# secondChoice/flink

Measured on AMD Instinct MI355X. Metric: records/sec/node, keyed TUMBLE SUM/COUNT/AVG at 1/2/4/8 GPU; % of HBM peak, higher is better.
Workload: dtype f64

## Files before the change

flink_amd/csrc/fg_kernels.hip:

```cpp
#include <hip/hip_runtime.h>

#include <algorithm>
#include <cstdio>
#include <vector>

#include <type_traits>

#include "fg_kernels.h"

namespace fg {

thread_local LaunchEvents g_launch_ev;

typedef long long RecV2 __attribute__((ext_vector_type(2)));
typedef const RecV2 __attribute__((address_space(1)))* GlobalRec;

__device__ __forceinline__ longlong2 ld2(const void* q) {
    const RecV2 v = *static_cast<const RecV2*>(q);
    return make_longlong2(v.x, v.y);
}
__device__ __forceinline__ void st2(void* q, longlong2 a) {
    RecV2 v;
    v.x = a.x;
    v.y = a.y;
// ... 3396 lines not shown
    int32_t t_base, ng;
    int32_t gk, wave, W;
    uint32_t* q;
    int32_t gsz;
    uint32_t xn[kTileTPL];
    uint32_t g_len[kTileTPL], g_st[kTileTPL], g_tot, b;
};
template <bool MAX>
__device__ __forceinline__ uint32_t dpp_op(uint32_t a, uint32_t b) { return MAX ? (a > b ? a : b) : a + b; }
template <bool MAX>
__device__ __forceinline__ uint32_t wave_incl_scan(uint32_t v) {
    v = dpp_op<MAX>(v, (uint32_t)__builtin_amdgcn_update_dpp(0, (int)v, 0x111, 0xf, 0xf, false));
    v = dpp_op<MAX>(v, (uint32_t)__builtin_amdgcn_update_dpp(0, (int)v, 0x112, 0xf, 0xf, false));
    v = dpp_op<MAX>(v, (uint32_t)__builtin_amdgcn_update_dpp(0, (int)v, 0x114, 0xf, 0xf, false));
    v = dpp_op<MAX>(v, (uint32_t)__builtin_amdgcn_update_dpp(0, (int)v, 0x118, 0xf, 0xf, false));
    v = dpp_op<MAX>(v, (uint32_t)__builtin_amdgcn_update_dpp(0, (int)v, 0x142, 0xa, 0xf, false));
    v = dpp_op<MAX>(v, (uint32_t)__builtin_amdgcn_update_dpp(0, (int)v, 0x143, 0xc, 0xf, false));
    return v;
}
__device__ __forceinline__ uint32_t wave_shr1(uint32_t v) {
    return (uint32_t)__builtin_amdgcn_update_dpp(0, (int)v, 0x138, 0xf, 0xf, false);
}

__device__ __forceinline__ int32_t tile_walk_grab(TileWalk& w, int lane) {
    if (!w.q) return w.wave + w.W * (w.gk++);
    uint32_t g = 0;
    if (lane == 0) g = atomicAdd(w.q, 1u);
    return (int32_t)__builtin_amdgcn_readfirstlane(g);
}
__device__ __forceinline__ void tile_walk_begin(TileWalk& w, const TilePass& tp, int32_t cb, int wave, int W,
                                                int lane, int32_t t_lo, int32_t t_hi, uint32_t* q = nullptr) {
    w.col = tp.dt + (int64_t)cb * tp.nt;
    w.rec = tp.rec;
    w.n = (uint32_t)tp.n;
    w.bad = false;
    w.nt = t_hi;
    const int32_t per = (t_hi - t_lo + W - 1) / W;
    w.gsz = per >= kTileGroup ? kTileGroup : (per + kTileTPL - 1) / kTileTPL * kTileTPL;
    if (w.gsz < kTileTPL) w.gsz = kTileTPL;
    w.t_base = t_lo;
    w.ng = t_hi > t_lo ? (t_hi - t_lo + w.gsz - 1) / w.gsz : 0;
    w.gk = 0;
    w.wave = wave;
    w.W = W;
    w.q = w.ng >= 4 * W ? q : nullptr;
    const int32_t g0 = tile_walk_grab(w, lane);
    w.tn = g0 < w.ng ? t_lo + g0 * w.gsz : t_hi;
#pragma unroll
    for (int q4 = 0; q4 < kTileTPL; q4++) {
        const int t = w.tn + lane * kTileTPL + q4;
        const bool ok = t < w.nt && lane * kTileTPL + q4 < w.gsz;
        const uint32_t x = gbl(w.col)[ok ? t : 0];
        w.xn[q4] = ok ? x : 0u;
        w.g_len[q4] = w.g_st[q4] = 0;
    }
    w.g_tot = w.b = 0;
}
__device__ __forceinline__ bool tile_walk_next(TileWalk& w, uint8_t* fm, uint32_t* dl, int lane,
                                               int32_t (&kr)[kTileRpl], int64_t (&vr)[kTileRpl], uint32_t& nrec) {
    static_assert(kTileRpl == 4, "one fragment-map word per lane");
    bool done = false;
    while (w.b >= w.g_tot) {
        w.t0 = w.tn;
        if (w.t0 >= w.nt) {
            done = true;
            break;
        }
        const int32_t gn = tile_walk_grab(w, lane);
        w.tn = gn < w.ng ? w.t_base + gn * w.gsz : w.nt;
        uint32_t base[kTileTPL], sum = 0;
#pragma unroll
        for (int q = 0; q < kTileTPL; q++) {
            const int t = w.t0 + lane * kTileTPL + q;
            const uint32_t x = w.xn[q];
            const int tn = w.tn + lane * kTileTPL + q;
            const bool okn = tn < w.nt && lane * kTileTPL + q < w.gsz;
            const uint32_t xn = gbl(w.col)[okn ? tn : 0];
            w.xn[q] = okn ? xn : 0u;
            w.g_len[q] = x >> 16;
            base[q] = (uint32_t)t * (uint32_t)kTileRecs + (x & 0xffffu);
            w.g_st[q] = sum;
            sum += w.g_len[q];
        }
        uint32_t inc = wave_incl_scan<false>(sum);
        asm volatile("" : "+v"(inc));
        const uint32_t ex = inc - sum;
        w.g_tot = (uint32_t)__builtin_amdgcn_readlane((int)inc, 63);
        w.b = 0;
        wave_lds_sync();
#pragma unroll
        for (int q = 0; q < kTileTPL; q++) {
            w.g_st[q] += ex;
            dl[lane * kTileTPL + q] = base[q] - w.g_st[q];
        }
    }
    if (done) {
        w.b = w.g_tot = 0;
    }
    uint32_t* fm32 = reinterpret_cast<uint32_t*>(fm);
    fm32[lane] = 0;
    wave_lds_sync();
#pragma unroll
    for (int q = 0; q < kTileTPL; q++) {
        const uint32_t st = w.g_st[q], len = w.g_len[q];
        if (len > 0 && st < w.b + kTileWin && st + len > w.b) fm[st > w.b ? st - w.b : 0] = (uint8_t)(lane * kTileTPL + q);
    }
    wave_lds_sync();
    const uint32_t e4 = fm32[lane];
    uint32_t e0 = e4 & 255u, e1 = (e4 >> 8) & 255u, e2 = (e4 >> 16) & 255u, e3 = e4 >> 24;
    e1 = e1 > e0 ? e1 : e0;
    e2 = e2 > e1 ? e2 : e1;
    e3 = e3 > e2 ? e3 : e2;
    const uint32_t pre = wave_shr1(wave_incl_scan<true>(e3));
    e0 = e0 > pre ? e0 : pre;
    e1 = e1 > pre ? e1 : pre;
    e2 = e2 > pre ? e2 : pre;
    e3 = e3 > pre ? e3 : pre;
    fm32[lane] = e0 | e1 << 8 | e2 << 16 | e3 << 24;
    wave_lds_sync();
    nrec = w.g_tot - w.b < (uint32_t)kTileWin ? w.g_tot - w.b : (uint32_t)kTileWin;
    uint32_t fq[kTileRpl], dq[kTileRpl];
#pragma unroll
    for (int u = 0; u < kTileRpl; u++) fq[u] = fm[lane + 64 * u] & (uint32_t)(kTileGroup - 1);
#pragma unroll
    for (int u = 0; u < kTileRpl; u++) dq[u] = dl[fq[u]];
#pragma unroll
    for (int u = 0; u < kTileRpl; u++) {
        const uint32_t jr = lane + 64 * u;
        uint32_t src = jr < nrec ? dq[u] + w.b + jr : 0u;
        if (src >= w.n) {
#ifdef FG_DEBUG_WALK
            if (!w.bad)
                printf("walk: lane %d u %d jr %u nrec %u b %u g_tot %u t0 %d nt %d n %u src %u fm %u dl %u "
                       "g_st %u %u g_len %u %u xn %u %u\n", lane, u, jr, nrec, w.b, w.g_tot, w.t0, w.nt, w.n, src,
                       (uint32_t)fm[jr], dl[fm[jr]], w.g_st[0], w.g_st[1], w.g_len[0], w.g_len[1], w.xn[0], w.xn[1]);
#endif
            w.bad = true;
            src = 0;
        }
#if defined(FG_DIAG_FIRE) && (FG_DIAG_FIRE & 1)
        kr[u] = (int32_t)((src * 2654435761u) >> 20);
        vr[u] = (int64_t)src;
#else
        const Rec12 r = ld_tile_rec(w.rec, (uint64_t)src);
        kr[u] = (int32_t)r.k;
        vr[u] = rec12_val(r);
#endif
    }
    w.b += kTileWin;
    return !done;
}

__global__ __launch_bounds__(256) void k_selftest_scan(const uint32_t* in, uint32_t* out) {
    const uint32_t v = in[threadIdx.x];
    const uint32_t a = wave_incl_scan<false>(v);
    const uint32_t m = wave_incl_scan<true>(v & 255u);
    out[3 * threadIdx.x] = a;
    out[3 * threadIdx.x + 1] = m;
    out[3 * threadIdx.x + 2] = wave_shr1(m);
}
__global__ __launch_bounds__(64) void k_selftest_walk(TilePass tp, uint32_t cap, uint32_t* out, uint32_t* n_out,
                                                      unsigned int* bad) {
    __shared__ __attribute__((aligned(16))) uint8_t s_fm[kTileWin];
    __shared__ uint32_t s_dl[kTileGroup];
    const int lane = threadIdx.x;
    const int32_t cb = blockIdx.x;
    TileWalk w;
    tile_walk_begin(w, tp, cb, 0, 1, lane, 0, tp.nt);
    int32_t kr[kTileRpl];
    int64_t vr[kTileRpl];
    uint32_t nrec = 0, pos = 0;
    while (tile_walk_next(w, s_fm, s_dl, lane, kr, vr, nrec)) {
#pragma unroll
        for (int u = 0; u < kTileRpl; u++) {
            const uint32_t jr = lane + 64 * u;
            if (jr < nrec && pos + jr < cap) out[(uint64_t)cb * cap + pos + jr] = (uint32_t)kr[u];
        }
        pos += nrec;
    }
    if (lane == 0) n_out[cb] = pos;
    if (__ballot(w.bad) != 0 && lane == 0) atomicOr(bad, 1u);
}
__global__ void k_selftest_fill(uint32_t* rec, uint64_t n) {
    for (uint64_t i = blockIdx.x * (uint64_t)blockDim.x + threadIdx.x; i < n; i += (uint64_t)gridDim.x * blockDim.x) {
        rec[3 * i] = (uint32_t)i;
        rec[3 * i + 1] = 0u;
        rec[3 * i + 2] = (uint32_t)i;
    }
}

int run_selftest(int device, char* msg, size_t cap_msg) {
    auto say = [&](const char* m) {
        if (msg && cap_msg) snprintf(msg, cap_msg, "%s", m);
    };
    if (hipSetDevice(device) != hipSuccess) {
        say("hipSetDevice failed");
        return 1;
    }
    uint64_t x = 0x5EEDF11Cull;
    auto rnd = [&]() {
        x = x * 6364136223846793005ull + 1442695040888963407ull;
        return (uint32_t)(x >> 33);
    };
    std::vector<uint32_t> in(256), got(3 * 256);
    for (auto& v : in) v = rnd() & 1023u;
    constexpr int NT = 300, NB = 3;
    std::vector<uint32_t> dt((size_t)NB * NT);
    std::vector<std::vector<uint32_t>> want(NB);
    for (int t = 0; t < NT; t++) {
        uint32_t off = rnd() % 64;
        for (int b = 0; b < NB; b++) {
            const uint32_t len = rnd() % 5 == 0 ? 0 : rnd() % 21;
            dt[(size_t)b * NT + t] = off | len << 16;
            for (uint32_t i = 0; i < len; i++) want[b].push_back((uint32_t)t * (uint32_t)kTileRecs + off + i);
            off += len;
        }
    }
    const uint64_t nrec = (uint64_t)NT * kTileRecs;
    uint32_t cap = 0;
    for (auto& v : want) cap = std::max<uint32_t>(cap, (uint32_t)v.size());
    void *d_in = nullptr, *d_out = nullptr, *d_rec = nullptr, *d_dt = nullptr, *d_w = nullptr, *d_n = nullptr,
         *d_bad = nullptr;
    int rc = 0;
    const char* what = nullptr;
    auto cleanup = [&]() {
        for (void* q : {d_in, d_out, d_rec, d_dt, d_w, d_n, d_bad})
            if (q) (void)hipFree(q);
    };
    if (hipMalloc(&d_in, 4 * 256) != hipSuccess || hipMalloc(&d_out, 4 * 3 * 256) != hipSuccess ||
        hipMalloc(&d_rec, 12 * nrec) != hipSuccess || hipMalloc(&d_dt, 4 * dt.size()) != hipSuccess ||
        hipMalloc(&d_w, 4 * (size_t)NB * cap + 4) != hipSuccess || hipMalloc(&d_n, 4 * NB) != hipSuccess ||
        hipMalloc(&d_bad, 4) != hipSuccess) {
        cleanup();
        say("self-check: device allocation failed");
        return 1;
    }
    (void)hipMemcpy(d_in, in.data(), 4 * 256, hipMemcpyHostToDevice);
    (void)hipMemcpy(d_dt, dt.data(), 4 * dt.size(), hipMemcpyHostToDevice);
    (void)hipMemset(d_bad, 0, 4);
    k_selftest_scan<<<1, 256>>>(static_cast<const uint32_t*>(d_in), static_cast<uint32_t*>(d_out));
    k_selftest_fill<<<256, 256>>>(static_cast<uint32_t*>(d_rec), nrec);
    TilePass tp{};
    tp.rec = d_rec;
    tp.dt = static_cast<const uint32_t*>(d_dt);
    tp.n = (int64_t)nrec;
    tp.nt = NT;
    tp.mt = NT;
    tp.nc = NB;
    k_selftest_walk<<<NB, 64>>>(tp, cap, static_cast<uint32_t*>(d_w), static_cast<uint32_t*>(d_n),
                                static_cast<unsigned int*>(d_bad));
    std::vector<uint32_t> walk((size_t)NB * cap), wn(NB);
    unsigned int bad = 0;
    if (hipDeviceSynchronize() != hipSuccess || hipMemcpy(got.data(), d_out, 4 * 3 * 256, hipMemcpyDeviceToHost) ||
        hipMemcpy(walk.data(), d_w, 4 * walk.size(), hipMemcpyDeviceToHost) ||
        hipMemcpy(wn.data(), d_n, 4 * NB, hipMemcpyDeviceToHost) || hipMemcpy(&bad, d_bad, 4, hipMemcpyDeviceToHost)) {
        cleanup();
        say("self-check: a kernel or copy failed");
        return 1;
    }
    cleanup();
    for (int wv = 0; wv < 4 && !what; wv++) {
        uint32_t a = 0, m = 0, prev = 0;
        for (int l = 0; l < 64; l++) {
            const uint32_t v = in[64 * wv + l];
            a += v;
            m = (v & 255u) > m ? (v & 255u) : m;
            const uint32_t* o = &got[3 * (64 * wv + l)];
            if (o[0] != a) what = "self-check: the DPP add scan (wave_incl_scan) is wrong";
            else if (o[1] != m) what = "self-check: the DPP max scan (wave_incl_scan) is wrong";
            else if (o[2] != (l ? prev : 0u)) what = "self-check: the DPP lane shift (wave_shr1) is wrong";
            if (what) break;
            prev = m;
        }
    }
    for (int b = 0; b < NB && !what; b++) {
        if (wn[b] != want[b].size()) what = "self-check: the tile walk visited a wrong number of records";
        for (size_t i = 0; !what && i < want[b].size(); i++)
            if (walk[(size_t)b * cap + i] != want[b][i]) what = "self-check: the tile walk read a wrong record";
    }
    if (!what && bad) what = "self-check: the tile walk addressed a record past its pass";
    if (what) {
        say(what);
        rc = 1;
    } else {
        say("ok");
    }
    return rc;
}

template <int VTC, bool TAB, int SM>
__global__ __launch_bounds__(kTileFireThreads) void k_tile_fire(TileFire fa) {
    const TileFire& f = fa;
    constexpr bool HOT = SM == 2;
    constexpr int T = kTileFireThreads, W = T / 64, S = kTileSlots;
    constexpr int kRounds = S / T + 1;
    static_assert(S % T == 0 && (S & (S - 1)) == 0, "table rounds");
    constexpr int kDummy = S + 1;
    __shared__ __attribute__((aligned(16))) int32_t t_key[S + 2];
    __shared__ uint32_t t_cs[S + 2];
    __shared__ unsigned long long t_v[S + 2];
    __shared__ __attribute__((aligned(16))) uint8_t s_fm[W][kTileWin];
    __shared__ uint32_t s_dl[W][kTileGroup];
    __shared__ uint32_t s_grp[kRounds * W];
    __shared__ uint16_t s_map[S + 1];
    __shared__ unsigned int s_flags;
    __shared__ uint32_t s_total;
    __shared__ unsigned long long s_out_base;
    __shared__ uint32_t s_rc[kTileMaxRegions];
    __shared__ uint32_t s_rb[kTileMaxRegions];
    __shared__ uint32_t s_gnext[kMaxTilePasses];
    const MergeParams& p = f.m;
    const bool dst = TAB && p.has_dst != 0;
    const int tid = threadIdx.x, lane = tid & 63, wave = tid >> 6;
#ifdef FG_STAMPS
    unsigned long long fst_acc[8] = {0, 0, 0, 0, 0, 0, 0, 0};
    unsigned long long fst_prev = __builtin_amdgcn_s_memtime();
#define FSTAMP(i)                                                     \
    do {                                                              \
        const unsigned long long now_ = __builtin_amdgcn_s_memtime(); \
        fst_acc[i] += now_ - fst_prev;                                \
        fst_prev = now_;                                              \
    } while (0)
#define FWAIT(kk, vv) asm volatile("" ::"v"(kk[kTileRpl - 1]), "v"(vv[kTileRpl - 1]))
#else
#define FSTAMP(i) \
    do {          \
    } while (0)
#define FWAIT(kk, vv) \
    do {              \
    } while (0)
#endif
    const int vt = VTC >= 0 ? VTC : p.val_type;
    const int64_t vinit = lds_repr(vt, val_identity(vt));
    const int sub = p.region_bits - f.tbits;
    const bool retry = p.retry_list != nullptr;
    const bool split = SM != 0 && f.split != 0;
    const bool merge = split && f.merge != 0;
    __shared__ int s_item;
    const int NI = retry ? p.n_retry
                   : merge ? (int)*gbl(f.sp.n_split)
                   : split ? (int)*gbl(f.sp.n_items)
                           : 1 << (f.tbits - kTileBits);
    const int G = gridDim.x;
    const bool xcd = !retry && !split && G % 8 == 0;
    for (int k = 0;; k++) {
        const int b = (int)blockIdx.x;
        int x = xcd ? k * G + (b % 8) * (G / 8) + b / 8 : b + k * G;
        if (split && !merge) {
            if (tid == 0) s_item = (int)atomicAdd(f.sp.next_item, 1u);
            __syncthreads();
            x = s_item;
            if (x >= NI) break;
        } else if (k * G >= NI) {
            break;
        }
        bool live = x < NI;
#if !defined(FG_FIRE_HOIST)
        const TileFire& f = (&fa)[opaque_zero()];
        const MergeParams& p = f.m;
#endif
        int r_lo = 0, r_hi = 0, item = 0;
        int32_t g_lo = 0, g_hi = 0x7fffffff, part = -1;
        int32_t mc0 = 0, mck = 0;
        if (live) {
            if (merge) {
                item = f.sp.split_b[x];
                mc0 = f.sp.split_c0[x];
                mck = f.sp.split_k[x];
                r_lo = item << (sub + kTileBits);
                r_hi = (item + 1) << (sub + kTileBits);
                live = *gbl(&f.sp.bfail[item]) == 0u;
            } else if (retry) {
                r_lo = gbl(p.retry_list)[x];
                r_hi = r_lo + 1;
                item = r_lo >> (sub + kTileBits);
            } else if (split) {
                const TileItem it = f.sp.items[x];
                item = it.bucket;
                g_lo = it.g_lo;
                g_hi = it.g_hi;
                part = it.part;
                r_lo = item << (sub + kTileBits);
                r_hi = (item + 1) << (sub + kTileBits);
            } else {
                item = x;
                r_lo = x << (sub + kTileBits);
                r_hi = (x + 1) << (sub + kTileBits);
            }
        }
        const bool to_part = split && !merge && part >= 0;
        for (int i = tid; i <= S + 1; i += T) {
            t_key[i] = kEmpty32;
            t_cs[i] = 0;
            t_v[i] = (unsigned long long)vinit;
        }
        if (TAB)
            for (int i = tid; i < kTileMaxRegions; i += T) s_rc[i] = 0;
        if (tid < kMaxTilePasses) s_gnext[tid] = 0;
        if (tid == 0) s_flags = 0;
        __syncthreads();
        FSTAMP(0);
        bool full = false;
#if defined(FG_DIAG_FIRE)
        uint64_t diag_sink = 0;
#endif
        auto slot_of = [&](int32_t key) -> int {
            if (key == kEmpty32) return S;
            uint32_t home = __umulhi((uint32_t)key * 0x9E3779B1u, (uint32_t)(S / 4)) * 4;
            for (int probe = 0; probe < S / 4; probe++) {
                const int4 q4 = *reinterpret_cast<const int4*>(&t_key[home]);
                const int32_t qq[4] = {q4.x, q4.y, q4.z, q4.w};
                int hit = -1, emp = -1;
#pragma unroll
                for (int z = 3; z >= 0; z--) {
                    if (qq[z] == key) hit = z;
                    if (qq[z] == kEmpty32) emp = z;
                }
                if (hit >= 0 && (emp < 0 || hit < emp)) return (int)home + hit;
                if (emp >= 0) {
                    const int old = atomicCAS(&t_key[home + emp], kEmpty32, key);
                    if (old == kEmpty32 || old == key) return (int)home + emp;
                    continue;
                }
                home = (home + 4) & (S - 1);
            }
            return -1;
        };
        if (TAB && p.n_src > 0 && !to_part) {
            constexpr int cap = kRegionCap;
            const int nreg = r_hi - r_lo, nrange = live ? p.n_src * nreg : 0;
            if (wave == 0) {
                constexpr int RPL = kTileMaxRegions / 64;
                uint32_t c[RPL], x = 0;
#pragma unroll
                for (int q = 0; q < RPL; q++) {
                    const int g = RPL * lane + q;
                    c[q] = g < nrange ? gbl(src_at(p, g / nreg).counts)[r_lo + g % nreg] : 0u;
                    x += c[q];
                }
                for (int off = 1; off < 64; off <<= 1) {
                    const uint32_t y = __shfl_up(x, off);
                    if (lane >= off) x += y;
                }
                uint32_t ex = x;
#pragma unroll
                for (int q = 0; q < RPL; q++) ex -= c[q];
#pragma unroll
                for (int q = 0; q < RPL; q++) {
                    if (RPL * lane + q < nrange) s_rb[RPL * lane + q] = ex;
                    ex += c[q];
                }
                if (lane == 63) s_total = x;
            }
            __syncthreads();
            const uint32_t NE = nrange ? s_total : 0u;
            for (uint32_t i0 = 0; !p.src_narrow && i0 < NE; i0 += kSrcU * T) {
                int64_t mk[kSrcU], cs[kSrcU], v[kSrcU];
#pragma unroll
                for (int u = 0; u < kSrcU; u++) {
                    const uint32_t i = i0 + u * T + tid;
                    mk[u] = cs[u] = v[u] = 0;
                    if (i >= NE) continue;
                    int lo = 0, hi = nrange;
                    while (hi - lo > 1) {
                        const int mid = (lo + hi) >> 1;
                        if (s_rb[mid] <= i) lo = mid;
                        else hi = mid;
                    }
                    const auto base = gbl(src_at(p, lo / nreg).base + (int64_t)(r_lo + lo % nreg) * 4 * cap);
                    const uint32_t e = i - s_rb[lo];
                    mk[u] = base[e];
                    cs[u] = base[cap + e];
                    v[u] = base[3 * cap + e];
                }
#pragma unroll
                for (int u = 0; u < kSrcU; u++) {
                    if (i0 + u * T + tid >= NE) continue;
                    const int sl = slot_of((int32_t)key_of(mk[u]));
                    if (sl < 0) {
                        full = true;
                        continue;
                    }
                    atomicAdd(&t_cs[sl], (uint32_t)cs[u]);
                    lds_val(&t_v[sl], v[u], vt, true);
                }
            }
            for (uint32_t i0 = 0; p.src_narrow && i0 < NE; i0 += kSrcU * T) {
                int64_t cs[kSrcU], v[kSrcU];
                int32_t mk[kSrcU];
#pragma unroll
                for (int u = 0; u < kSrcU; u++) {
                    const uint32_t i = i0 + u * T + tid;
                    mk[u] = 0;
                    cs[u] = v[u] = 0;
                    if (i >= NE) continue;
                    int lo = 0, hi = nrange;
                    while (hi - lo > 1) {
                        const int mid = (lo + hi) >> 1;
                        if (s_rb[mid] <= i) lo = mid;
                        else hi = mid;
                    }
                    const TableRef sr = src_at(p, lo / nreg);
                    const auto base = gbl(sr.base + (int64_t)(r_lo + lo % nreg) * 4 * cap);
                    const uint32_t e = i - s_rb[lo];
                    const bool nar = sr.narrow != 0;
                    mk[u] = tab_key32(base, cap, e, nar);
                    cs[u] = tab_cs(base, cap, e, nar);
                    v[u] = tab_v(base, cap, e, nar);
                }
#pragma unroll
                for (int u = 0; u < kSrcU; u++) {
                    if (i0 + u * T + tid >= NE) continue;
                    const int sl = slot_of(mk[u]);
                    if (sl < 0) {
                        full = true;
                        continue;
                    }
                    atomicAdd(&t_cs[sl], (uint32_t)cs[u]);
                    lds_val(&t_v[sl], v[u], vt, true);
                }
            }
        }
        FSTAMP(4);
        if (live && merge) {
            constexpr int kPartU = 4;
            for (int c0 = mc0; c0 < mc0 + mck; c0 += kTileMaxRegions) {
                const int nc = min(kTileMaxRegions, mc0 + mck - c0);
                __syncthreads();
                if (wave == 0) {
                    constexpr int RPL = kTileMaxRegions / 64;
                    uint32_t c[RPL], x = 0;
#pragma unroll
                    for (int q = 0; q < RPL; q++) {
                        const int g = RPL * lane + q;
                        c[q] = 0;
                        if (g < nc) {
                            const uint32_t off = f.sp.part_off[c0 + g], n = f.sp.part_n[c0 + g];
                            if ((uint64_t)off + n <= (uint64_t)f.sp.part_cap) c[q] = n;
                            else atomicOr(p.overflow, 2u);
                        }
                        x += c[q];
                    }
                    for (int off = 1; off < 64; off <<= 1) {
                        const uint32_t y = __shfl_up(x, off);
                        if (lane >= off) x += y;
                    }
                    uint32_t ex = x;
#pragma unroll
                    for (int q = 0; q < RPL; q++) ex -= c[q];
#pragma unroll
                    for (int q = 0; q < RPL; q++) {
                        if (RPL * lane + q < nc) s_rb[RPL * lane + q] = ex;
                        ex += c[q];
                    }
                    if (lane == 63) s_total = x;
                }
                __syncthreads();
                const uint32_t NE = s_total;
                for (uint32_t i0 = 0; i0 < NE; i0 += kPartU * T) {
                    int32_t pk[kPartU];
                    uint32_t pc[kPartU];
                    unsigned long long pv[kPartU];
#pragma unroll
                    for (int u = 0; u < kPartU; u++) {
                        const uint32_t i = i0 + u * T + tid;
                        pk[u] = kEmpty32;
                        pc[u] = 0;
                        pv[u] = 0;
                        if (i >= NE) continue;
                        int lo = 0, hi = nc;
                        while (hi - lo > 1) {
                            const int mid = (lo + hi) >> 1;
                            if (s_rb[mid] <= i) lo = mid;
                            else hi = mid;
                        }
                        const uint32_t e = f.sp.part_off[c0 + lo] + (i - s_rb[lo]);
                        pk[u] = f.sp.p_key[e];
                        pc[u] = f.sp.p_cs[e];
                        pv[u] = f.sp.p_v[e];
                    }
#pragma unroll
                    for (int u = 0; u < kPartU; u++) {
                        if (i0 + u * T + tid >= NE) continue;
                        const int sl = slot_of(pk[u]);
                        if (sl < 0) {
                            full = true;
                            continue;
                        }
                        atomicAdd(&t_cs[sl], pc[u]);
                        lds_val(&t_v[sl], lds_repr(vt, (int64_t)pv[u]), vt, true);
                    }
                }
            }
        } else if (live) {
            auto insert_plain = [&](auto FULL, auto RETRY, const int32_t (&kr)[kTileRpl], const int64_t (&vr)[kTileRpl],
                                    uint32_t nrec) {
#if defined(FG_DIAG_FIRE) && (FG_DIAG_FIRE & 2)
#pragma unroll
                for (int u = 0; u < kTileRpl; u++)
                    if (lane + 64 * u < nrec) diag_sink ^= (uint64_t)kr[u] ^ (uint64_t)vr[u];
                return;
#endif
                uint32_t hm[kTileRpl];
                int4 bq[kTileRpl];
#pragma unroll
                for (int u = 0; u < kTileRpl; u++) {
                    hm[u] = __umulhi((uint32_t)kr[u] * 0x9E3779B1u, (uint32_t)(S / 4)) * 4;
                    bq[u] = *reinterpret_cast<const int4*>(&t_key[hm[u]]);
                }
#pragma unroll
                for (int u = 0; u < kTileRpl; u++) {
                    if (!decltype(FULL)::value && lane + 64 * u >= nrec) continue;
                    const int32_t key = kr[u];
                    if (decltype(RETRY)::value && retry &&
                        (int)((uint64_t)mix_of((int64_t)key) >> (64 - p.region_bits)) != r_lo)
                        continue;
                    int sl = -1;
                    if (key == kEmpty32) {
                        sl = S;
                    } else {
                        uint32_t home = hm[u];
                        int4 q4 = bq[u];
                        for (int probe = 0; probe < S / 4; probe++) {
                            const int32_t qq[4] = {q4.x, q4.y, q4.z, q4.w};
                            int hit = -1, emp = -1;
#pragma unroll
                            for (int z = 3; z >= 0; z--) {
                                if (qq[z] == key) hit = z;
                                if (qq[z] == kEmpty32) emp = z;
                            }
                            if (hit >= 0 && (emp < 0 || hit < emp)) {
                                sl = (int)home + hit;
                                break;
                            }
                            if (emp >= 0) {
                                const int old = atomicCAS(&t_key[home + emp], kEmpty32, key);
                                if (old == kEmpty32 || old == key) {
                                    sl = (int)home + emp;
                                    break;
                                }
                            } else {
                                home = (home + 4) & (S - 1);
                            }
                            q4 = *reinterpret_cast<const int4*>(&t_key[home]);
                        }
                    }
                    if (sl < 0) {
                        full = true;
                        continue;
                    }
                    atomicAdd(&t_cs[sl], 1u);
                    lds_val(&t_v[sl], vr[u], vt, true);
                }
            };
            auto insert_hot = [&](const int32_t (&kr)[kTileRpl], const int64_t (&vr)[kTileRpl], uint32_t nrec) {
                const bool hot = vt >= 0 && vt <= 2;
                uint32_t hm[kTileRpl];
                int4 bq[kTileRpl];
                int sl[kTileRpl];
                uint32_t cn[kTileRpl];
                int64_t va[kTileRpl];
#pragma unroll
                for (int u = 0; u < kTileRpl; u++) {
                    hm[u] = __umulhi((uint32_t)kr[u] * 0x9E3779B1u, (uint32_t)(S / 4)) * 4;
                    bq[u] = *reinterpret_cast<const int4*>(&t_key[hm[u]]);
                    cn[u] = 1u;
                    va[u] = vr[u];
                }
                bool pend[kTileRpl];
#pragma unroll
                for (int u = 0; u < kTileRpl; u++) {
                    const int32_t key = kr[u];
                    bool valid = lane + 64 * u < (int)nrec;
                    if (retry) valid = valid && (int)((uint64_t)mix_of((int64_t)key) >> (64 - p.region_bits)) == r_lo;
                    if (hot) {
                        const int32_t k0 = __builtin_amdgcn_readfirstlane(key);
                        const bool mine = valid && key == k0;
                        const uint64_t m = __ballot(mine);
                        if (__popcll(m) >= 16) {
                            int64_t sv = mine ? vr[u] : 0;
#pragma unroll
                            for (int off = 32; off > 0; off >>= 1) {
                                const int64_t o = __shfl_xor(sv, off);
                                if (vt == 2) sv = __double_as_longlong(__longlong_as_double(sv) + __longlong_as_double(o));
                                else sv += o;
                            }
                            const int leader = __ffsll((long long)m) - 1;
                            if (mine) {
                                if (lane == leader) {
                                    cn[u] = (uint32_t)__popcll(m);
                                    va[u] = sv;
                                } else {
                                    valid = false;
                                }
                            }
                        }
                    }
                    const int4 q4 = bq[u];
                    int z = q4.w == key ? 3 : -1;
                    z = q4.z == key ? 2 : z;
                    z = q4.y == key ? 1 : z;
                    z = q4.x == key ? 0 : z;
                    int s0 = z >= 0 ? (int)hm[u] + z : -1;
                    s0 = key == kEmpty32 ? S : s0;
                    pend[u] = valid && s0 < 0;
                    sl[u] = valid ? s0 : kDummy;
                }
#pragma unroll
                for (int u = 0; u < kTileRpl; u++) {
                    if (__ballot(pend[u]) == 0) continue;
                    if (!pend[u]) continue;
                    const int32_t key = kr[u];
                    uint32_t home = hm[u];
                    int4 q4 = bq[u];
                    int found = -1;
                    for (int probe = 0; probe < S / 4 && found < 0; probe++) {
                        const int32_t qq[4] = {q4.x, q4.y, q4.z, q4.w};
                        int hit = -1, emp = -1;
#pragma unroll
                        for (int z = 3; z >= 0; z--) {
                            if (qq[z] == key) hit = z;
                            if (qq[z] == kEmpty32) emp = z;
                        }
                        if (hit >= 0 && (emp < 0 || hit < emp)) {
                            found = (int)home + hit;
                        } else if (emp >= 0) {
                            const int old = atomicCAS(&t_key[home + emp], kEmpty32, key);
                            if (old == kEmpty32 || old == key) found = (int)home + emp;
                            else q4 = *reinterpret_cast<const int4*>(&t_key[home]);
                        } else {
                            home = (home + 4) & (S - 1);
                            q4 = *reinterpret_cast<const int4*>(&t_key[home]);
                        }
                    }
                    if (found < 0) full = true;
                    sl[u] = found >= 0 ? found : kDummy;
                }
#pragma unroll
                for (int u = 0; u < kTileRpl; u++) {
                    atomicAdd(&t_cs[sl[u]], cn[u]);
                    lds_val(&t_v[sl[u]], va[u], vt, true);
                }
            };
            auto insert = [&](const int32_t (&kr)[kTileRpl], const int64_t (&vr)[kTileRpl], uint32_t nrec) {
                if constexpr (HOT) {
                    insert_hot(kr, vr, nrec);
                } else {
#if defined(FG_INSERT_GENERIC)
                    insert_plain(std::false_type{}, std::true_type{}, kr, vr, nrec);
#else
                    if (retry) insert_plain(std::false_type{}, std::true_type{}, kr, vr, nrec);
                    else if (nrec == (uint32_t)kTileWin) insert_plain(std::true_type{}, std::false_type{}, kr, vr, nrec);
                    else insert_plain(std::false_type{}, std::false_type{}, kr, vr, nrec);
#endif
                }
            };
            for (int pi = 0; pi < f.n_passes; pi++) {
                const TilePass tp = tile_pass(f, pi);
                int32_t t_lo = 0, t_hi = tp.nt;
                if (split) {
                    t_lo = g_lo - f.sp.gpre[pi] > 0 ? g_lo - f.sp.gpre[pi] : 0;
                    t_hi = g_hi - f.sp.gpre[pi] < tp.nt ? g_hi - f.sp.gpre[pi] : tp.nt;
                    if (t_lo >= t_hi) continue;
                }
                TileWalk w;
                tile_walk_begin(w, tp, (tp.lane << (f.tbits - kTileBits)) | item, wave, W, lane, t_lo, t_hi,
#if defined(FG_WALK_STATIC)
                                nullptr);
#else
                                pi < kMaxTilePasses ? &s_gnext[pi] : nullptr);
#endif
                int32_t ka[kTileRpl], kb[kTileRpl];
                int64_t va[kTileRpl], vb[kTileRpl];
                uint32_t na = 0, nb = 0;
                bool more = tile_walk_next(w, s_fm[wave], s_dl[wave], lane, ka, va, na);
                FSTAMP(1);
                while (more) {
                    const bool hb = tile_walk_next(w, s_fm[wave], s_dl[wave], lane, kb, vb, nb);
                    FSTAMP(1);
                    FWAIT(ka, va);
                    FSTAMP(2);
                    insert(ka, va, na);
                    FSTAMP(3);
                    if (!hb) break;
                    more = tile_walk_next(w, s_fm[wave], s_dl[wave], lane, ka, va, na);
                    FSTAMP(1);
                    FWAIT(kb, vb);
                    FSTAMP(2);
                    insert(kb, vb, nb);
                    FSTAMP(3);
                }
                if (__ballot(w.bad) != 0 && lane == 0) atomicOr(p.overflow, 8u);
            }
        }
        if (full) atomicOr(&s_flags, 4u);
#if defined(FG_DIAG_FIRE)
        if (diag_sink == 0x5EEDull) atomicOr(p.overflow, 0u);
#endif
        FSTAMP(4);
        __syncthreads();
        FSTAMP(5);
        {
#if !defined(FG_FIRE_HOIST)
        const TileFire& f = (&fa)[opaque_zero()];
        const MergeParams& p = f.m;
#endif
        uint32_t occ_mask = 0;
        auto region_of = [&](int slot) -> int {
            const int64_t key = slot == S ? (int64_t)kEmpty32 : (int64_t)t_key[slot];
            return (int)((uint64_t)mix_of(key) >> (64 - p.region_bits)) - r_lo;
        };
#pragma unroll
        for (int r = 0; r < kRounds; r++) {
            const int slot = r < kRounds - 1 ? r * T + tid : S;
            const bool occ = (r < kRounds - 1 || tid == 0) && t_cs[slot] != 0;
            const uint64_t bal = __ballot(occ);
            if (occ) occ_mask |= 1u << r;
            if (lane == 0) s_grp[r * W + wave] = (uint32_t)__popcll(bal);
            if (dst && !to_part && occ && live) atomicAdd(&s_rc[region_of(slot)], 1u);
        }
        __syncthreads();
        if (wave == 0) {
            constexpr int NG = kRounds * W;
            constexpr int GPL = (NG + 63) / 64;
            uint32_t gv[GPL], xs = 0;
#pragma unroll
            for (int q = 0; q < GPL; q++) {
                gv[q] = GPL * lane + q < NG ? s_grp[GPL * lane + q] : 0u;
                xs += gv[q];
            }
            for (int off = 1; off < 64; off <<= 1) {
                const uint32_t y = __shfl_up(xs, off);
                if (lane >= off) xs += y;
            }
            uint32_t ex = xs;
#pragma unroll
            for (int q = 0; q < GPL; q++) ex -= gv[q];
#pragma unroll
            for (int q = 0; q < GPL; q++) {
                if (GPL * lane + q < NG) s_grp[GPL * lane + q] = ex;
                ex += gv[q];
            }
            const uint32_t total = __shfl(xs, 63);
            bool over = false;
            if (dst && !to_part)
                for (int q = lane; q < r_hi - r_lo; q += 64) over = over || s_rc[q] > (uint32_t)kRegionCap;
            over = __ballot(over) != 0;
            if (lane == 0) {
                unsigned int fl = s_flags | (over ? 4u : 0u);
                if (live && !(fl & 4u) && !to_part && (!TAB || p.emit)) {
                    const unsigned long long ob = atomicAdd(p.out_count, (unsigned long long)total);
                    s_out_base = ob;
                    if ((int64_t)(ob + total) > p.out_cap) fl |= 2u;
                }
                if (live && !(fl & 4u) && to_part) {
                    const uint32_t ob = atomicAdd(f.sp.part_fill, total);
                    s_out_base = ob;
                    if ((uint64_t)ob + total > (uint64_t)f.sp.part_cap) fl |= 2u;
                    f.sp.part_off[part] = ob;
                    f.sp.part_n[part] = total;
                }
                if (live && to_part && (fl & 4u)) f.sp.part_n[part] = kChunkFailed;
                s_flags = fl;
                s_total = total;
                if (fl) atomicOr(p.overflow, fl);
                if (live && (fl & 4u) && p.fail_list && (!to_part || atomicExch(&f.sp.bfail[item], 1u) == 0u)) {
                    const uint32_t nr = (uint32_t)(r_hi - r_lo);
                    const uint32_t at = atomicAdd(p.fail_n, nr);
                    for (uint32_t q = 0; q < nr; q++)
                        if (at + q < (uint32_t)p.fail_cap)
                            p.fail_list[at + q] = ((uint32_t)p.job << kFailJobShift) | (uint32_t)(r_lo + (int)q);
                }
            }
        }
        __syncthreads();
        const unsigned int fl = s_flags;
#pragma unroll
        for (int r = 0; r < kRounds; r++) {
            const bool occ = (occ_mask >> r) & 1;
            const uint64_t bal = __ballot(occ);
            if (occ) s_map[s_grp[r * W + wave] + (uint32_t)__popcll(bal & ((1ull << lane) - 1))] =
                (uint16_t)(r < kRounds - 1 ? r * T + tid : S);
        }
        __syncthreads();
        FSTAMP(6);
        if (live && to_part && !(fl & 6u)) {
            const uint32_t total = s_total;
            const uint32_t ob = (uint32_t)s_out_base;
            for (uint32_t i = tid; i < total; i += T) {
                const int sl = s_map[i];
                f.sp.p_key[ob + i] = sl == S ? kEmpty32 : t_key[sl];
                f.sp.p_cs[ob + i] = t_cs[sl];
                f.sp.p_v[ob + i] = t_v[sl];
            }
        } else if (live && (!TAB || p.emit) && !(fl & 6u)) {
            const uint32_t total = s_total;
            const unsigned long long ob = s_out_base;
            for (uint32_t i = tid; i < total; i += T) {
                const int sl = s_map[i];
                const int64_t v = lds_repr(vt, (int64_t)t_v[sl]);
                write_row_k<TAB>(p, ob + i, sl == S ? (int64_t)kEmpty32 : (int64_t)t_key[sl], t_cs[sl], 0ull, &v, vt);
            }
        }
        if (TAB && dst && live && !to_part && !(fl & 5u)) {
            constexpr int cap = kRegionCap;
            const int nreg = r_hi - r_lo;
            __syncthreads();
            if (wave == 0) {
                constexpr int RPL = kTileMaxRegions / 64;
                uint32_t c[RPL], x = 0;
#pragma unroll
                for (int q = 0; q < RPL; q++) {
                    c[q] = RPL * lane + q < nreg ? s_rc[RPL * lane + q] : 0u;
                    x += c[q];
                }
                for (int off = 1; off < 64; off <<= 1) {
                    const uint32_t y = __shfl_up(x, off);
                    if (lane >= off) x += y;
                }
                uint32_t ex = x;
#pragma unroll
                for (int q = 0; q < RPL; q++) ex -= c[q];
#pragma unroll
                for (int q = 0; q < RPL; q++) {
                    const int rr = RPL * lane + q;
                    if (rr < nreg) {
                        const uint32_t old = p.dst.counts[r_lo + rr];
                        p.dst.counts[r_lo + rr] = c[q];
                        if (p.dst_total) atomicAdd(p.dst_total, (unsigned long long)((int64_t)c[q] - (int64_t)old));
                        s_rb[rr] = ex;
                        s_rc[rr] = ex;
                    }
                    ex += c[q];
                }
            }
            __syncthreads();
#pragma unroll
            for (int r = 0; r < kRounds; r++) {
                if (!((occ_mask >> r) & 1)) continue;
                const int slot = r < kRounds - 1 ? r * T + tid : S;
                s_map[atomicAdd(&s_rc[region_of(slot)], 1u)] = (uint16_t)slot;
            }
            __syncthreads();
            const uint32_t total = s_total;
            for (uint32_t i = tid; i < total; i += T) {
                int lo = 0, hi = nreg;
                while (hi - lo > 1) {
                    const int mid = (lo + hi) >> 1;
                    if (s_rb[mid] <= i) lo = mid;
                    else hi = mid;
                }
                const int sl = s_map[i];
                const uint32_t at = i - s_rb[lo];
                int64_t* db = p.dst.base + (int64_t)(r_lo + lo) * 4 * cap;
                const int32_t k32 = sl == S ? kEmpty32 : t_key[sl];
                if (p.dst.narrow) {
                    reinterpret_cast<int32_t*>(db)[at] = k32;
                    reinterpret_cast<uint32_t*>(db)[cap + at] = t_cs[sl];
                    db[cap + at] = lds_repr(vt, (int64_t)t_v[sl]);
                } else {
                    db[at] = mix_of((int64_t)k32);
                    db[cap + at] = (int64_t)t_cs[sl];
                    db[2 * cap + at] = 0;
                    db[3 * cap + at] = lds_repr(vt, (int64_t)t_v[sl]);
                }
            }
        }
        }
        __syncthreads();
        FSTAMP(7);
    }
#ifdef FG_STAMPS
    if (fa.m.stamps && lane == 0)
        for (int i = 0; i < 8; i++) atomicAdd(&fa.m.stamps[i], fst_acc[i]);
#endif
#undef FSTAMP
#undef FWAIT
}

hipError_t launch_tile_fire(const TileFire& f, int32_t workgroups, hipStream_t s) {
    if (f.n_passes < 1 || f.tbits < kTileBits || f.m.region_bits < f.tbits || f.m.mv) return hipErrorInvalidValue;
    if (f.m.has_dst || f.m.n_src > 0) {
        if (f.m.src_null_mask) return hipErrorInvalidValue;
        const int sub = kTileBits + f.m.region_bits - f.tbits;
        if (!f.m.retry_list && sub > kTileMaxRegionBits) return hipErrorInvalidValue;
        const int64_t nreg = f.m.retry_list ? 1 : (int64_t)1 << sub;
        if ((int64_t)f.m.n_src * nreg > kTileMaxRegions) return hipErrorInvalidValue;
    }
    const dim3 g((unsigned)workgroups), b(kTileFireThreads);
    const bool tab = f.m.has_dst || f.m.n_src > 0;
    if (f.split && !f.merge && !f.sp.next_item) return hipErrorInvalidValue;
    if (f.merge && (!f.split || !f.sp.split_b || !f.sp.n_split)) return hipErrorInvalidValue;
    const bool hot = f.hot && f.split && !f.merge && f.m.val_type >= 0 && f.m.val_type <= 2;
    const int sm = !f.split ? 0 : hot ? 2 : 1;
#define FG_TILE_FIRE_SM(V, TB)                                                     \
    do {                                                                           \
        if (sm == 0) fg_launch((k_tile_fire<V, TB, 0>), g, b, 0, s, f);            \
        else if (sm == 1) fg_launch((k_tile_fire<V, TB, 1>), g, b, 0, s, f);       \
        else fg_launch((k_tile_fire<V, TB, 2>), g, b, 0, s, f);                    \
    } while (0)
#define FG_TILE_FIRE(V)                          \
    do {                                         \
        if (tab) FG_TILE_FIRE_SM(V, true);       \
        else FG_TILE_FIRE_SM(V, false);          \
    } while (0)
    switch (f.m.val_type) {
        case 2: FG_TILE_FIRE(2); break;
        case 1: FG_TILE_FIRE(1); break;
        case 0: FG_TILE_FIRE(0); break;
        default: FG_TILE_FIRE(-1); break;
    }
#undef FG_TILE_FIRE
#undef FG_TILE_FIRE_SM
    return hipGetLastError();
}

constexpr int kTilePlanThreads = 1024;
__global__ __launch_bounds__(kTilePlanThreads) void k_tile_plan(TileFire f) {
    __shared__ uint32_t s_wave[kTilePlanThreads / 64];
    const TileSplit& sp = f.sp;
    const int nb = 1 << (f.tbits - kTileBits);
    const int tid = threadIdx.x;
    const int32_t G = sp.gpre[f.n_passes];
    constexpr int BPT = kMaxTileBuckets / kTilePlanThreads;
    uint32_t kk[BPT], tb[BPT], mine = 0, nitem = 0, nsplit = 0, nchunk = 0;
#pragma unroll
    for (int q = 0; q < BPT; q++) {
        const int bk = tid * BPT + q;
        tb[q] = 0;
        if (bk >= nb) continue;
        for (int pi = 0; pi < f.n_passes; pi++) {
            const TilePass tp = tile_pass(f, pi);
            if (tp.btot) tb[q] += gbl(tp.btot)[(tp.lane << (f.tbits - kTileBits)) | bk];
        }
        mine += tb[q];
    }
    uint32_t lane_total;
    (void)block_exclusive_scan(mine, s_wave, &lane_total);
    const uint64_t chunk = sp.chunk ? (uint64_t)sp.chunk : max((uint64_t)kTileChunk, (uint64_t)lane_total / (uint64_t)nb);
#pragma unroll
    for (int q = 0; q < BPT; q++) {
        const int bk = tid * BPT + q;
        kk[q] = 0;
        if (bk >= nb) continue;
        uint64_t k = tb[q] > chunk ? (tb[q] + chunk - 1) / chunk : 1;
        if (k > (uint64_t)G) k = G > 0 ? (uint64_t)G : 1;
        kk[q] = (uint32_t)k;
        nitem += (uint32_t)k;
        if (k > 1) {
            nsplit++;
            nchunk += (uint32_t)k;
        }
    }
    uint32_t t_item, t_split, t_chunk;
    const uint32_t b_item = block_exclusive_scan(nitem, s_wave, &t_item);
    const uint32_t b_split = block_exclusive_scan(nsplit, s_wave, &t_split);
    const uint32_t b_chunk = block_exclusive_scan(nchunk, s_wave, &t_chunk);
    const bool fits = t_item <= (uint32_t)sp.max_items && t_split <= (uint32_t)sp.max_split;
    if (tid == 0) {
        *sp.n_items = fits ? t_item : 0u;
        *sp.n_split = fits ? t_split : 0u;
        if (!fits) atomicOr(f.m.overflow, 2u);
    }
    if (!fits) return;
    uint32_t it = b_item, si = b_split, ci = b_chunk;
#pragma unroll
    for (int q = 0; q < BPT; q++) {
        const int bk = tid * BPT + q;
        const uint32_t k = kk[q];
        if (k == 0) continue;
        if (k > 1) {
            sp.split_b[si] = bk;
            sp.split_c0[si] = (int32_t)ci;
            sp.split_k[si] = (int32_t)k;
            sp.bfail[bk] = 0u;
            si++;
        }
        for (uint32_t c = 0; c < k; c++) {
            TileItem x;
            x.bucket = bk;
            x.g_lo = k > 1 ? (int32_t)((int64_t)G * c / k) : 0;
            x.g_hi = k > 1 ? (int32_t)((int64_t)G * (c + 1) / k) : G;
            x.part = k > 1 ? (int32_t)(ci + c) : -1;
            sp.items[it + c] = x;
        }
        it += k;
        if (k > 1) ci += k;
    }
}

hipError_t launch_tile_plan(const TileFire& f, hipStream_t s) {
    if (!f.split || f.n_passes < 1 || f.n_passes > kMaxTilePasses || (1 << (f.tbits - kTileBits)) > kMaxTileBuckets ||
        !f.sp.items || !f.sp.n_items || !f.sp.split_b || !f.sp.n_split || !f.sp.bfail)
        return hipErrorInvalidValue;
    fg_launch(k_tile_plan, dim3(1), dim3(kTilePlanThreads), 0, s, f);
    return hipGetLastError();
// ... 99 lines not shown
```

Before: 67.68 billion.

## Queue hash-probe misses per wave and drain them in full-wave batches

In the plain tile-fire insert path (non-table, SM==0), each record first checks only its home 4-slot bucket with branch-free selects. Records that miss are compacted by ballot into a per-wave LDS queue carved out of s_map. The queue is drained 64 at a time through the full slot_of probe, so divergent probe loops run with full lanes instead of a few stragglers per step. This adds LDS traffic, wave syncs, and reuse of s_map as scratch, which relies on s_map not being live during insertion.

```diff
diff --git a/flink_amd/csrc/fg_kernels.hip b/flink_amd/csrc/fg_kernels.hip
--- a/flink_amd/csrc/fg_kernels.hip
+++ b/flink_amd/csrc/fg_kernels.hip
@@ -3722,7 +3722,9 @@
     __shared__ __attribute__((aligned(16))) uint8_t s_fm[W][kTileWin];
     __shared__ uint32_t s_dl[W][kTileGroup];
     __shared__ uint32_t s_grp[kRounds * W];
-    __shared__ uint16_t s_map[S + 1];
+    __shared__ __attribute__((aligned(16))) uint16_t s_map[S + 1];
+    constexpr int kQueueBytes = 2 * S / W, kQueueCap = kQueueBytes / 12;
+    static_assert(kQueueBytes % 8 == 0 && kQueueCap >= 64, "a wave's miss queue takes a whole record step");
     __shared__ unsigned int s_flags;
     __shared__ uint32_t s_total;
     __shared__ unsigned long long s_out_base;
@@ -4013,6 +4015,23 @@
                 }
             }
         } else if (live) {
+            constexpr bool QUEUE = !TAB && SM == 0;
+            uint32_t qn = 0;
+            unsigned long long* const q_val = reinterpret_cast<unsigned long long*>(s_map) + wave * (kQueueBytes / 8);
+            int32_t* const q_key = reinterpret_cast<int32_t*>(q_val + kQueueCap);
+            auto drain = [&](uint32_t c) {
+                wave_lds_sync();
+                qn -= c;
+                if ((uint32_t)lane < c) {
+                    const int sl = slot_of(q_key[qn + lane]);
+                    if (sl < 0) {
+                        full = true;
+                    } else {
+                        atomicAdd(&t_cs[sl], 1u);
+                        lds_val(&t_v[sl], (int64_t)q_val[qn + lane], vt, true);
+                    }
+                }
+            };
             auto insert_plain = [&](auto FULL, auto RETRY, const int32_t (&kr)[kTileRpl], const int64_t (&vr)[kTileRpl],
                                     uint32_t nrec) {
 #if defined(FG_DIAG_FIRE) && (FG_DIAG_FIRE & 2)
@@ -4030,47 +4049,77 @@
                 }
 #pragma unroll
                 for (int u = 0; u < kTileRpl; u++) {
-                    if (!decltype(FULL)::value && lane + 64 * u >= nrec) continue;
-                    const int32_t key = kr[u];
-                    if (decltype(RETRY)::value && retry &&
-                        (int)((uint64_t)mix_of((int64_t)key) >> (64 - p.region_bits)) != r_lo)
-                        continue;
-                    int sl = -1;
-                    if (key == kEmpty32) {
-                        sl = S;
-                    } else {
-                        uint32_t home = hm[u];
-                        int4 q4 = bq[u];
-                        for (int probe = 0; probe < S / 4; probe++) {
-                            const int32_t qq[4] = {q4.x, q4.y, q4.z, q4.w};
-                            int hit = -1, emp = -1;
-#pragma unroll
-                            for (int z = 3; z >= 0; z--) {
-                                if (qq[z] == key) hit = z;
-                                if (qq[z] == kEmpty32) emp = z;
-                            }
-                            if (hit >= 0 && (emp < 0 || hit < emp)) {
-                                sl = (int)home + hit;
-                                break;
-                            }
-                            if (emp >= 0) {
-                                const int old = atomicCAS(&t_key[home + emp], kEmpty32, key);
-                                if (old == kEmpty32 || old == key) {
-                                    sl = (int)home + emp;
+                    if constexpr (!QUEUE) {
+                        if (!decltype(FULL)::value && lane + 64 * u >= nrec) continue;
+                        const int32_t key = kr[u];
+                        if (decltype(RETRY)::value && retry &&
+                            (int)((uint64_t)mix_of((int64_t)key) >> (64 - p.region_bits)) != r_lo)
+                            continue;
+                        int sl = -1;
+                        if (key == kEmpty32) {
+                            sl = S;
+                        } else {
+                            uint32_t home = hm[u];
+                            int4 q4 = bq[u];
+                            for (int probe = 0; probe < S / 4; probe++) {
+                                const int32_t qq[4] = {q4.x, q4.y, q4.z, q4.w};
+                                int hit = -1, emp = -1;
+#pragma unroll
+                                for (int z = 3; z >= 0; z--) {
+                                    if (qq[z] == key) hit = z;
+                                    if (qq[z] == kEmpty32) emp = z;
+                                }
+                                if (hit >= 0 && (emp < 0 || hit < emp)) {
+                                    sl = (int)home + hit;
                                     break;
                                 }
-                            } else {
-                                home = (home + 4) & (S - 1);
+                                if (emp >= 0) {
+                                    const int old = atomicCAS(&t_key[home + emp], kEmpty32, key);
+                                    if (old == kEmpty32 || old == key) {
+                                        sl = (int)home + emp;
+                                        break;
+                                    }
+                                } else {
+                                    home = (home + 4) & (S - 1);
+                                }
+                                q4 = *reinterpret_cast<const int4*>(&t_key[home]);
                             }
-                            q4 = *reinterpret_cast<const int4*>(&t_key[home]);
                         }
+                        if (sl < 0) {
+                            full = true;
+                            continue;
+                        }
+                        atomicAdd(&t_cs[sl], 1u);
+                        lds_val(&t_v[sl], vr[u], vt, true);
+                    } else {
+                        const int32_t key = kr[u];
+                        bool valid = decltype(FULL)::value || lane + 64 * u < nrec;
+                        if (decltype(RETRY)::value && retry)
+                            valid = valid && (int)((uint64_t)mix_of((int64_t)key) >> (64 - p.region_bits)) == r_lo;
+                        const int4 q4 = bq[u];
+                        int z = q4.w == key ? 3 : -1;
+                        z = q4.z == key ? 2 : z;
+                        z = q4.y == key ? 1 : z;
+                        z = q4.x == key ? 0 : z;
+                        int sl = z >= 0 ? (int)hm[u] + z : -1;
+                        sl = key == kEmpty32 ? S : sl;
+                        if (valid && sl >= 0) {
+                            atomicAdd(&t_cs[sl], 1u);
+                            lds_val(&t_v[sl], vr[u], vt, true);
+                        }
+                        const bool miss = valid && sl < 0;
+                        const uint64_t bal = __ballot(miss);
+                        if (bal == 0) continue;
+                        const uint32_t m = (uint32_t)__popcll(bal);
+                        if (qn + m > (uint32_t)kQueueCap) drain(qn);
+                        if (miss) {
+                            const uint32_t at = qn + (uint32_t)__popcll(bal & ((1ull << lane) - 1));
+                            q_val[at] = (unsigned long long)vr[u];
+                            q_key[at] = key;
+                        }
+                        qn += m;
+                        if (qn >= 64u) drain(64u);
                     }
-                    if (sl < 0) {
-                        full = true;
-                        continue;
-                    }
-                    atomicAdd(&t_cs[sl], 1u);
-                    lds_val(&t_v[sl], vr[u], vt, true);
                 }
             };
             auto insert_hot = [&](const int32_t (&kr)[kTileRpl], const int64_t (&vr)[kTileRpl], uint32_t nrec) {
@@ -4212,6 +4261,10 @@
                 }
                 if (__ballot(w.bad) != 0 && lane == 0) atomicOr(p.overflow, 8u);
             }
+            if constexpr (QUEUE) {
+                while (qn != 0) drain(qn < 64u ? qn : 64u);
+                FSTAMP(3);
+            }
         }
         if (full) atomicOr(&s_flags, 4u);
 #if defined(FG_DIAG_FIRE)
```

Result: faster. 71.25 billion, median of 6 (+5.3%).
